# theogf/AugmentedGaussianProcesses.jl

Measured on AMD Instinct MI355X. Metric: cavi_iters_per_sec, higher is better.
Workload: dtype f64

## Files before the change

### augmentedgaussianprocesses.jl_amd/csrc/agp_chol.h

```cpp
#pragma once
#include "agp_cavi.h"
#include "agp_device.h"

namespace agp {

constexpr int LDP = TILE + 2;
constexpr int CHOL_THREADS = 512;

__device__ __forceinline__ double rcp1(double p) {
  double r = __builtin_amdgcn_rcp(p);
  return fma(r, fma(-p, r, 1.0), r);
}
__device__ __forceinline__ double rsqrt1(double p) {
  double y = __builtin_amdgcn_rsq(p);
  const double h = 0.5 * p;
  y = y * fma(-h * y, y, 1.5);
  y = y * fma(-h * y, y, 1.5);
  return y;
}
__device__ __forceinline__ float rsqrt1(float p) {
  float y = __builtin_amdgcn_rsqf(p);
  const float h = 0.5f * p;
  y = y * fmaf(-h * y, y, 1.5f);
  return y;
// ... 953 lines not shown

__global__ void k_wait_ge_fast(const int32_t* __restrict__ p, int32_t want, int32_t* __restrict__ info) {
  if (threadIdx.x != 0) return;
  long spins = 0;
  while ((int32_t)(__hip_atomic_load(p, __ATOMIC_RELAXED, __HIP_MEMORY_SCOPE_SYSTEM) - want) < 0) {
    __builtin_amdgcn_s_sleep(8);
    if (++spins > (1L << 27)) {
      atomicExch(info, -2);
      break;
    }
  }
}

__device__ __forceinline__ void dag_signal(int32_t* flag, int32_t epoch) {
  __builtin_amdgcn_fence(__ATOMIC_RELEASE, "workgroup");
  __syncthreads();
  if (threadIdx.x == 0) __hip_atomic_store(flag, epoch, __ATOMIC_RELAXED, __HIP_MEMORY_SCOPE_AGENT);
}

template <typename T>
__device__ __forceinline__ typename Mfma<T>::acc_t mma_tile16(const T* Ar, const T* Bc, int kend,
                                                              typename Mfma<T>::acc_t acc, bool neg, int lane) {
  const T* pa = Ar + (lane & 15) * LDP + (lane >> 4);
  const T* pb = Bc + (lane & 15) * LDP + (lane >> 4);
  typename Mfma<T>::acc_t p1;
#pragma unroll
  for (int r = 0; r < 4; ++r) p1[r] = T(0);
#pragma unroll 2
  for (int kk = 0; kk < kend / 4; kk += 2) {
    T a0 = pa[kk * 4], a1 = pa[kk * 4 + 4];
    const T b0 = pb[kk * 4], b1 = pb[kk * 4 + 4];
    if (neg) {
      a0 = -a0;
      a1 = -a1;
    }
    acc = Mfma<T>::mma(a0, b0, acc);
    p1 = Mfma<T>::mma(a1, b1, p1);
  }
#pragma unroll
  for (int r = 0; r < 4; ++r) acc[r] += p1[r];
  return acc;
}

template <typename T, typename F>
__device__ __forceinline__ void subst_tile(T* Ts, T* Xs, T* G, F after_first) {
  typedef typename Mfma<T>::acc_t acc_t;
  const int lane = threadIdx.x & 63, wave = threadIdx.x >> 6, ri = wave & 3, cj = wave >> 2;
  T* rowt = Ts + 16 * ri * LDP;
  T* own1 = rowt + 16 * cj;
  T* own2 = own1 + 32;
  const T* xlow = Xs + (32 + 16 * cj) * LDP;
  T* urow = Xs + 16 * (ri & 1) * LDP + 32 * (ri >> 1);
  auto emit = [&](int col0, acc_t v) {
    if (G) {
#pragma unroll
      for (int r = 0; r < 4; ++r)
        __hip_atomic_store(G + (16 * ri + Mfma<T>::row(lane, r)) * TILE + col0 + (lane & 15), v[r], __ATOMIC_RELAXED,
                           __HIP_MEMORY_SCOPE_AGENT);
    }
  };
  acc_t a;
#pragma unroll
  for (int r = 0; r < 4; ++r) a[r] = T(0);
  a = mma_tile16<T>(rowt, Xs + 16 * cj * LDP, 16 * (cj + 1), a, false, lane);
  after_first();
  acc_store16<T>(own1, a, lane);
  emit(16 * cj, a);
  __syncthreads();
  a = acc_load16<T>(own2, lane);
  a = mma_tile16<T>(rowt, xlow, 32, a, true, lane);
  acc_store16<T>(urow + 16 * cj, a, lane);
  __syncthreads();
#pragma unroll
  for (int r = 0; r < 4; ++r) a[r] = T(0);
  a = mma_tile16<T>(urow, xlow + 32, 16 * (cj + 1), a, false, lane);
  acc_store16<T>(own2, a, lane);
  emit(32 + 16 * cj, a);
}

template <typename T>
constexpr bool dag_feed_deferred() {
  return sizeof(T) == 8;
}
template <typename T, bool DEFER = dag_feed_deferred<T>()>
struct ChainPrefetch {
  const T* src;
  T *dT, *dD;
  int* bad;
  const int32_t *f1, *f2;
  int32_t epoch;
  int* ok;
  const T* dgsrc;
  T* gDg;
  const T* lsrc;
  T* gL;
  int ld_i;
  bool coh = false;
  int test = 0;
  T v[TILE * TILE / 256];
  __device__ __forceinline__ void operator()(int round) {
    int t = (int)threadIdx.x - 256;
    if (t < 0) return;
    if (sizeof(T) == 8) asm volatile("" : "+v"(t));
    if (round < 2) {
      if (dgsrc) {
#pragma unroll
        for (int q = 0; q < TILE * TILE / 512; ++q) {
          const int e = t + (2 * q + round) * 256;
          if (coh) __hip_atomic_store(gDg + e, dgsrc[(e >> 6) * LDP + (e & 63)], __ATOMIC_RELAXED, __HIP_MEMORY_SCOPE_AGENT);
          else gDg[e] = dgsrc[(e >> 6) * LDP + (e & 63)];
        }
      }
      return;
    }
    if (round < 4 && lsrc) {
#pragma unroll
      for (int q = 0; q < TILE * TILE / 512; ++q) {
        const int e = t + (2 * q + (round - 2)) * 256;
        gL[(e >> 6) * ld_i + (e & 63)] = lsrc[(e >> 6) * LDP + (e & 63)];
      }
    }
    if (!src) return;
    if (round == 3) {
      if (t == 0)
        *ok = (__hip_atomic_load(f1, __ATOMIC_RELAXED, __HIP_MEMORY_SCOPE_AGENT) == epoch) &&
              (__hip_atomic_load(f2, __ATOMIC_RELAXED, __HIP_MEMORY_SCOPE_AGENT) == epoch) && !(test & 2);
      return;
    }
    if (round < 4 || round > 6 || !*ok) return;
    if (round >= 5) {
      T* d = round == 5 ? dT : dD;
#pragma unroll
      for (int q = 0; q < TILE * TILE / 256; ++q) {
        const int e = t + q * 256;
        if (is_sent<T>(v[q])) *bad = 1;
        d[(e >> 6) * LDP + (e & 63)] = v[q];
      }
    }
    if (round <= 5) {
      const T* g = round == 4 ? src : src + TILE * TILE;
#pragma unroll
      for (int q = 0; q < TILE * TILE / 256; ++q)
        v[q] = __hip_atomic_load(g + t + q * 256, __ATOMIC_RELAXED, __HIP_MEMORY_SCOPE_AGENT);
    }
  }
  static __device__ __forceinline__ unsigned sent_away(T x) {
    typedef typename Sent<T>::U U;
    return (unsigned)(__builtin_bit_cast(U, x) >> (8 * sizeof(U) - 32)) ^ (unsigned)(Sent<T>::bits >> (8 * sizeof(U) - 32));
  }
  template <int HB>
  __device__ __forceinline__ void half(int rr) {
    if (!DEFER) {
      (*this)(HB + rr);
      return;
    }
    int t = (int)threadIdx.x - 256;
    if (t < 0) return;
    asm volatile("" : "+v"(t));
    if (HB == 0) {
      if (rr < 2) {
        if (dgsrc) {
#pragma unroll
          for (int q = 0; q < TILE * TILE / 512; ++q) {
            const int e = t + (2 * q + rr) * 256;
            if (coh) __hip_atomic_store(gDg + e, dgsrc[(e >> 6) * LDP + (e & 63)], __ATOMIC_RELAXED, __HIP_MEMORY_SCOPE_AGENT);
            else gDg[e] = dgsrc[(e >> 6) * LDP + (e & 63)];
          }
        }
        return;
      }
      if (lsrc) {
#pragma unroll
        for (int q = 0; q < TILE * TILE / 512; ++q) {
          const int e = t + (2 * q + (rr - 2)) * 256;
          gL[(e >> 6) * ld_i + (e & 63)] = lsrc[(e >> 6) * LDP + (e & 63)];
        }
      }
      if (src && rr == 3 && t == 0)
        *ok = (__hip_atomic_load(f1, __ATOMIC_RELAXED, __HIP_MEMORY_SCOPE_AGENT) == epoch) &&
              (__hip_atomic_load(f2, __ATOMIC_RELAXED, __HIP_MEMORY_SCOPE_AGENT) == epoch) && !(test & 2);
      return;
    }
    if (!src || (rr != 0 && rr != 3) || !*ok) return;
    if (rr == 3) {
      T* d = dT + (t >> 6) * LDP + (t & 63);
      unsigned away = ~0u;
#pragma unroll
      for (int q = 0; q < TILE * TILE / 256; ++q) {
        away = min(away, sent_away(v[q]));
        d[q * 4 * LDP] = v[q];
      }
      if (away == 0) *bad = 1;
    }
    const T* g = rr == 0 ? src : src + TILE * TILE;
#pragma unroll
    for (int q = 0; q < TILE * TILE / 256; ++q)
      v[q] = __hip_atomic_load(g + t + q * 256, __ATOMIC_RELAXED, __HIP_MEMORY_SCOPE_AGENT);
  }
  __device__ __forceinline__ void store_d() {
    int t = (int)threadIdx.x - 256;
    if (t < 0) return;
    asm volatile("" : "+v"(t));
    const T* g = src + TILE * TILE + t;
    const bool again = (test & 1) != 0;
    unsigned away = ~0u;
#pragma unroll
    for (int q = 0; q < TILE * TILE / 256; ++q) away = min(away, sent_away(v[q]));
    T* d = dD + (t >> 6) * LDP + (t & 63);
    if (away == 0 || again) {
#pragma unroll
      for (int q = 0; q < TILE * TILE / 256; ++q)
        d[q * 4 * LDP] = hv_settle<T>(g + q * 256, again ? __builtin_bit_cast(T, Sent<T>::bits) : v[q]);
    } else {
#pragma unroll
      for (int q = 0; q < TILE * TILE / 256; ++q) d[q * 4 * LDP] = v[q];
    }
  }
};

typedef unsigned int u32x4 __attribute__((ext_vector_type(4)));
__device__ __forceinline__ u32x4 load16_sc1(const void* p) {
  u32x4 v;
  asm volatile("global_load_dwordx4 %0, %1, off sc1" : "=v"(v) : "v"(p) : "memory");
  return v;
}
__device__ __forceinline__ void wait_vmcnt0() { asm volatile("s_waitcnt vmcnt(0)" ::: "memory"); }
template <typename T>
__device__ __forceinline__ T vec16_elem(u32x4 v, int i);
template <>
__device__ __forceinline__ double vec16_elem<double>(u32x4 v, int i) {
  const unsigned long long u = ((unsigned long long)v[2 * i + 1] << 32) | v[2 * i];
  return __builtin_bit_cast(double, u);
}
template <>
__device__ __forceinline__ float vec16_elem<float>(u32x4 v, int i) {
  return __builtin_bit_cast(float, (unsigned int)v[i]);
}
template <typename T>
__device__ __forceinline__ int pro_slot_off(int tid, int e) {
  constexpr int VEC = 16 / (int)sizeof(T);
  return (e / VEC) * (CHOL_THREADS * VEC) + tid * VEC + (e % VEC);
}

template <typename T>
struct EpiArgs {
  int on = 0;
  int64_t B = 0;
  int nslices = 0;
  const T* pk = nullptr;
  int64_t ldp = 0;
  T kdiag = T(0);
  const T* kd_ptr = nullptr;
  int use_kt = 0;
  T jitter = T(0), rho = T(0);
  LikParams<T> lp{};
  const T* y = nullptr;
  const int64_t* idx = nullptr;
  T *Kt = nullptr, *muf = nullptr, *varf = nullptr, *cb = nullptr, *theta = nullptr, *r = nullptr, *w = nullptr;
  int* flags = nullptr;
  const T* lam = nullptr;
  T* gamma = nullptr;
};

// ... 61 lines not shown
    }
#pragma unroll
    for (int r = 0; r < 4; ++r) red[wave * 256 + Mfma<T>::row(lane, r) * 16 + (lane & 15)] = acc[r];
    __syncthreads();
    if (threadIdx.x < 256) {
      const int e = threadIdx.x;
      T v = red[e];
#pragma unroll
      for (int o = 1; o < NW; ++o) v += red[o * 256 + e];
      out[(int64_t)(sl * PRO_PRE_KS + q) * TILE * TILE + (16 * bi + (e >> 4)) * TILE + 16 * bj + (e & 15)] = v;
    }
    __syncthreads();
  }
}

constexpr int ARRIVE_STRIDE = 16;
__device__ __forceinline__ void pro_arrival_gate(const int32_t* arrive, int g, int32_t want, int32_t* info) {
  if (threadIdx.x == 0) {
    long spins = 0;
    while ((int32_t)(__hip_atomic_load(arrive + g * ARRIVE_STRIDE, __ATOMIC_RELAXED, __HIP_MEMORY_SCOPE_AGENT) - want) < 0) {
      __builtin_amdgcn_s_sleep(8);
      if (++spins > (1L << 23)) {
        atomicExch(info, -4);
        break;
      }
    }
  }
  __syncthreads();
  __builtin_amdgcn_fence(__ATOMIC_ACQUIRE, "agent");
}

constexpr int PRO_NEAR = 4;
__host__ __device__ __forceinline__ int64_t pro_nhelp(int64_t nt, int64_t c, int ks, int kf) {
  const int64_t ntc = nt - c, nn = ntc < PRO_NEAR ? ntc : PRO_NEAR;
  return nn * (kf - 1) + (ntc - nn) * (ks - 1);
}
template <typename T>
__device__ __forceinline__ void pro_slice(const T* __restrict__ kap, int64_t ldk, const T* __restrict__ w, int64_t R0, int64_t c0,
                                          int64_t q0, int64_t q1, T* sm, Acc8<T>& acc) {
  constexpr int Q = TILE * TILE / CHOL_THREADS;
  const int r = threadIdx.x & 63, kb = threadIdx.x >> 6;
  const bool dg = R0 == c0;
  T va[Q], vb[Q], wv[Q];
  auto ldg = [&](int64_t qc) {
    const T* __restrict__ p = kap + (qc * TILE) * ldk;
#pragma unroll
    for (int q = 0; q < Q; ++q) {
      const int k = kb + 8 * q;
      va[q] = p[k * ldk + R0 + r];
      vb[q] = dg ? T(0) : p[k * ldk + c0 + r];
      wv[q] = w[qc * TILE + k];
    }
  };
  if (q0 < q1) ldg(q0);
  int cur = 0;
  for (int64_t qc = q0; qc < q1; ++qc) {
    T* As = sm + cur * 2 * TILE * LDP;
    T* Bs = As + TILE * LDP;
#pragma unroll
    for (int q = 0; q < Q; ++q) {
      const int k = kb + 8 * q;
      As[r * LDP + k] = va[q] * wv[q];
      Bs[r * LDP + k] = dg ? va[q] : vb[q];
    }
    __syncthreads();
    if (qc + 1 < q1) ldg(qc + 1);
    mma8<T>(As, Bs, acc);
    cur ^= 1;
  }
  __syncthreads();
}

constexpr long long CHAIN_GO_TICKS = 4LL * 100000000LL;
#ifndef AGP_TILES_WAVES_F64
#define AGP_TILES_WAVES_F64 4
#endif
#ifndef AGP_TILES_WAVES_F32
#define AGP_TILES_WAVES_F32 6
#endif
template <typename T, bool STEP, bool BATCH>
constexpr bool dag_block_subst() {
  return STEP && !BATCH && sizeof(T) == 8;
}
template <typename T, int ROLE, bool PRO>
constexpr int dag_min_waves() {
  return ROLE != 2 ? 1 : PRO ? (sizeof(T) == 8 ? 2 : 4) : (sizeof(T) == 8 ? AGP_TILES_WAVES_F64 : AGP_TILES_WAVES_F32);
}
template <typename T>
struct ProdArgs {
  T* out = nullptr;
  int64_t ld = 0;
  int64_t base = 0;
  T* fill = nullptr;
  int64_t fill_n = 0;
  double* ld_out = nullptr;
  int32_t* status = nullptr;
};

constexpr int STRACE_SLOTS = 8192, STRACE_XPUB = 600, STRACE_EXT = 1100, STRACE_FILL0 = 1400, STRACE_FILL1 = 1500, STRACE_WG0 = 2048,
              STRACE_WG1 = 4096, STRACE_MAXWG = 2048, STRACE_SAFE0 = 6144, STRACE_SAFE1 = 6400;
#ifdef AGP_STEP_TRACE
struct StraceExit {
  unsigned long long* p;
  __device__ ~StraceExit() {
    if (p && threadIdx.x == 0) *p = wall_clock64();
  }
};
#define STRACE(i) \
  if (PRO && ROLE == 0 && trace && threadIdx.x == 0) trace[i] = wall_clock64()
#else
#define STRACE(i)
#endif

template <typename T, bool FUSED, bool BATCH = false, bool TRACE = false, bool STEP = false, bool PRO = false, int ROLE = 0>
__global__ __launch_bounds__(CHOL_THREADS, (dag_min_waves<T, ROLE, PRO>()))
void k_chol_dag(CholBatch<T> bt, int nb, int64_t fstride, int64_t ld, int64_t ldx,
                                                           int64_t lde, int64_t ne, int64_t nt,
                                                           int32_t* __restrict__ info, int64_t nvalid, int32_t* flags,
                                                           int32_t epoch, unsigned long long* trace, T* H, int64_t hstride,
                                                           int64_t nx_, const T* __restrict__ erow, int opts, DagSync sync,
                                                           ProArgs<T> pro = ProArgs<T>{}, EpiArgs<T> epi = EpiArgs<T>{},
                                                           ProdArgs<T> prod = ProdArgs<T>{}) {
  static_assert(!PRO || (FUSED && !BATCH), "the prologue exists for single-problem launches with a chain workgroup only");
  static_assert(ROLE == 0 || (FUSED && STEP && !TRACE), "the split launch exists for the CAVI step's launches");
  const int64_t nx = STEP ? 0 : nx_;
  constexpr bool SUBST = dag_block_subst<T, STEP, BATCH>();
  const int write_x = STEP ? 0 : (opts & 1);
  const bool store_l = STEP ? false : (opts & 2) != 0;
  const int prob = BATCH ? (int)(blockIdx.x % (unsigned)nb) : 0;
  const int64_t bidx = BATCH ? (int64_t)(blockIdx.x / (unsigned)nb) : (int64_t)blockIdx.x;
  T* A = bt.A[prob];
  T* X = bt.X[prob];
  T* __restrict__ Dg = bt.Dg[prob];
  T* E = bt.E[prob];
  if (BATCH) erow = bt.R[prob];
  flags += prob * fstride;
  constexpr int64_t SLOT = TILE * TILE;
  T* HX = H + prob * hstride;
  T* HP = HX + nt * SLOT;
  T* HL = HP + 2 * nt * SLOT;
  __shared__ __attribute__((aligned(16))) T sm[((FUSED && ROLE != 2) || PRO ? 4 : 2) * TILE * LDP];
  __shared__ __attribute__((aligned(16))) T sc[(ROLE == 2 && !PRO) ? TILE : SC_ELEMS];
  __shared__ T piv[TILE];
  __shared__ int wait_ok, pf_ok, pf_bad;
  if (ROLE == 1) {
    if (threadIdx.x == 0) {
      wait_ok = 1;
      if (sync.here) __hip_atomic_fetch_add(sync.here, 1, __ATOMIC_RELAXED, __HIP_MEMORY_SCOPE_SYSTEM);
      unsigned spins = 0;
      const long long t0 = (long long)wall_clock64();
      while (sync.go) {
        const int32_t d = (int32_t)(__hip_atomic_load(sync.go, __ATOMIC_RELAXED, __HIP_MEMORY_SCOPE_SYSTEM) - sync.go_val);
        if (d == 0) break;
        if (d > 0) {
          wait_ok = 0;
          break;
        }
        __builtin_amdgcn_s_sleep(4);
        if ((++spins & 1023u) == 0 && (long long)wall_clock64() - t0 > CHAIN_GO_TICKS) {
          atomicExch(info, -1);
          wait_ok = 0;
#ifdef AGP_DEBUG_PTRS
          atomicAdd(&agp_dag_diag[5], 1ull);
#endif
          break;
        }
      }
    }
    __syncthreads();
    if (!wait_ok) {
      chain_count_out(sync);
      return;
    }
    __builtin_amdgcn_fence(__ATOMIC_ACQUIRE, "agent");
  }
  T* bufA = sm;
  T* bufB = sm + TILE * LDP;
  const int tid = threadIdx.x;
#ifdef AGP_STEP_TRACE
  StraceExit strace_exit{(PRO && ROLE == 0 && trace && bidx < STRACE_MAXWG) ? trace + STRACE_WG1 + bidx : nullptr};
  if (bidx < STRACE_MAXWG) STRACE(STRACE_WG0 + bidx);
#endif
  int64_t b = bidx, c = 0;
  bool helper = false;
  int64_t hbase = 0;
  const bool is_prod = !BATCH && !STEP && ROLE != 1 && prod.out != nullptr && bidx >= prod.base;
  static_assert(ROLE == 0 || STEP, "product workgroups (ProdArgs) must reach their sentinel refill unconditionally: ROLE 0 only");
  if (is_prod) {
    b = 0;
  } else if (PRO && ROLE == 1) {
  } else if (PRO) {
    for (;;) {
      if (c == nt) {
        const T sv = __builtin_bit_cast(T, Sent<T>::bits);
        if (b < 64) STRACE(STRACE_FILL0 + b);
        for (int64_t i = b * CHOL_THREADS + tid; i < pro.fill_n; i += (int64_t)pro.nfill * CHOL_THREADS) pro.fill[i] = sv;
        if (b < 64) STRACE(STRACE_FILL1 + b);
        return;
      }
      const int64_t nh = pro_nhelp(nt, c, pro.ks[c], pro.kf[c]), ntile = nt - c + ne + (nx ? c + 1 : 0);
      if (b < nh) {
        helper = true;
        break;
      }
      b -= nh;
      if (b < ntile) break;
      b -= ntile;
      hbase += nh;
      ++c;
// ... 36 lines not shown
  T* rowp = idr ? nullptr : ext ? E + (R - nt) * TILE * lde : A + R * TILE * ld;
  const int64_t ldr = ext ? lde : ld, c0 = c * TILE;
  int32_t* ready = flags;
  int32_t* xready = flags + (nt + ne + nx) * nt * DAG_FS;
  int32_t* pre1 = xready + nt * DAG_FS;
  int32_t* pre2 = pre1 + nt * DAG_FS;
  int32_t* abortf = pre2 + nt * DAG_FS;
#define DAG_TR(slot) \
  if (TRACE && tid == 0) trace[bidx * 8 + (slot)] = wall_clock64()
#define DAG_TRC(col, slot) \
  if (TRACE && tid == 0) trace[chain_slot(col, nt, ne, nx) * 8 + (slot)] = wall_clock64()
  if (is_prod) {
    const int64_t pidx = bidx - prod.base, nprod = nt * (nt + 1) / 2;
    if (prod.fill) {
      const T sv = __builtin_bit_cast(T, Sent<T>::bits);
      for (int64_t i = pidx * CHOL_THREADS + tid; i < prod.fill_n; i += nprod * CHOL_THREADS) prod.fill[i] = sv;
    }
    int64_t pi, pj;
    tri_index(pidx, pi, pj);
    const bool pdiag = pi == pj;
    const int64_t Ri = nt + ne + pi, Rj = nt + ne + pj;
    Acc8<T> pacc;
    pacc.zero();
    for (int64_t k = pi; k < nt; ++k) {
      if (!dag_wait(ready + (Ri * nt + k) * DAG_FS, pdiag ? nullptr : ready + (Rj * nt + k) * DAG_FS, epoch, abortf, info, &wait_ok))
        return;
      if (pdiag) load_tile_lds_hv<T>(HL + (Ri * nt + k) * SLOT, bufA);
      else load_tiles_lds_hv2<T>(HL + (Ri * nt + k) * SLOT, bufA, HL + (Rj * nt + k) * SLOT, bufB);
      __syncthreads();
      mma8<T>(bufA, pdiag ? bufA : bufB, pacc);
      __syncthreads();
    }
    const int64_t i0 = pi * TILE, j0 = pj * TILE;
    if (pdiag) {
      acc8_foreach<T>(pacc, [&](int r, int cc, T& val) { bufA[r * LDP + cc] = val; });
      __syncthreads();
      acc8_foreach<T>(pacc, [&](int r, int cc, T& val) {
        prod.out[(i0 + r) * prod.ld + i0 + cc] = cc > r ? bufA[cc * LDP + r] : val;
      });
    } else {
      acc8_foreach<T>(pacc, [&](int r, int cc, T& val) {
        prod.out[(i0 + r) * prod.ld + j0 + cc] = val;
        prod.out[(j0 + cc) * prod.ld + i0 + r] = val;
      });
    }
    if (prod.ld_out && pidx == nprod - 1) {
      __syncthreads();
      double lsum = 0.0;
      for (int64_t i = tid; i < nvalid; i += CHOL_THREADS) {
        const T* px = HX + (i / TILE) * SLOT + (i % TILE) * (TILE + 1);
        const T xv = hv_settle<T>(px, __hip_atomic_load(px, __ATOMIC_RELAXED, __HIP_MEMORY_SCOPE_AGENT));
        lsum -= log((double)xv);
      }
      lsum = block_sum<double>(lsum, reinterpret_cast<double*>(sc));
      if (tid == 0) {
        prod.ld_out[0] = lsum;
        int32_t* st_ = prod.status;
        if (st_) {
          const int32_t i0_ = __hip_atomic_load(st_, __ATOMIC_RELAXED, __HIP_MEMORY_SCOPE_AGENT);
          const int32_t i1_ = __hip_atomic_load(st_ + 1, __ATOMIC_RELAXED, __HIP_MEMORY_SCOPE_AGENT);
          const int32_t i2_ = __hip_atomic_load(st_ + 2, __ATOMIC_RELAXED, __HIP_MEMORY_SCOPE_AGENT);
          if (i1_ != 0 && st_[3] == 0) st_[3] = (i0_ != 0 || i2_ != 0) ? 2 : 1;
        }
      }
    }
    return;
  }
  DAG_TR(0);
  const bool chain = FUSED && c == 0 && b == 0;
  if (STEP && !BATCH && sync.started && chain && tid == 0 && ROLE != 1)
    __hip_atomic_store(sync.started, sync.seq, __ATOMIC_RELAXED, __HIP_MEMORY_SCOPE_SYSTEM);
  if (ROLE == 2 && chain) {
    if (tid == 0 && sync.go) __hip_atomic_store(sync.go, sync.go_val, __ATOMIC_RELAXED, __HIP_MEMORY_SCOPE_SYSTEM);
    if (!PRO) return;
  }
  if (ROLE == 1 && !chain) return;
  Acc8<T> acc;
  if (PRO && ROLE == 1) {
  } else if (PRO && !ext) {
    const int64_t ntc_ = nt - c, nn_ = ntc_ < PRO_NEAR ? ntc_ : PRO_NEAR;
    const bool pre = pro_pre_on<T>() && pro.pre && pro_pre_tile(R, c);
    const int ksc = pre ? 1 : b < nn_ ? pro.kf[c] : pro.ks[c];
    const int64_t nq = pro.Kdim / TILE;
    const int tsb = chain ? 0 : (R < 4 && c < 4) ? 64 + 8 * (4 * (int)R + (int)c) : 2040;
    PRO_TS(tsb);
    acc.zero();
    if (pre && pro.pre[PRO_PRE_VALID] == T(1)) {
      const T* __restrict__ pp = pro.pre + (R + c) * PRO_PRE_KS * TILE * TILE;
      T pv[PRO_PRE_KS][8];
      int e = 0;
      acc8_foreach<T>(acc, [&](int r, int cc, T& val) {
        (void)val;
#pragma unroll
        for (int q = 0; q < PRO_PRE_KS; ++q) pv[q][e] = pp[q * TILE * TILE + r * TILE + cc];
        ++e;
      });
      e = 0;
      acc8_foreach<T>(acc, [&](int r, int cc, T& val) {
        (void)r;
        (void)cc;
        T v = pv[0][e];
#pragma unroll
        for (int q = 1; q < PRO_PRE_KS; ++q) v += pv[q][e];
        val = v;
        ++e;
      });
    } else {
      pro_slice<T>(pro.kap, pro.ldk, pro.w, R * TILE, c0, 0, nq / ksc, sm, acc);
    }
    if (pro.packed) {
      if (pro.arrive) pro_arrival_gate(pro.arrive, pro.grp[c], pro.arrive_want, info);
      const T* __restrict__ tp = pro.packed + pack_index(R, c, nt) * (TILE * TILE);
      acc8_foreach<T>(acc, [&](int r, int cc, T& val) { val = tp[r * TILE + cc]; });
    }
    PRO_TS(tsb + 1);
    Acc8<T> e2v, kiv;
    acc8_foreach<T>(e2v, [&](int r, int cc, T& val) { val = pro.eta2[(R * TILE + r) * pro.ldm + c0 + cc]; });
    acc8_foreach<T>(kiv, [&](int r, int cc, T& val) { val = pro.Kinv[(R * TILE + r) * pro.ldm + c0 + cc]; });
    if (ksc > 1) {
      const int64_t h0 = hbase + (b < nn_ ? b * (pro.kf[c] - 1) : nn_ * (pro.kf[c] - 1) + (b - nn_) * (pro.ks[c] - 1));
      if (tid < ksc - 1) {
        long spins = 0;
        while (__hip_atomic_load(pro.sflags + (h0 + tid) * DAG_FS, __ATOMIC_RELAXED, __HIP_MEMORY_SCOPE_AGENT) != epoch) {
          __builtin_amdgcn_s_sleep(1);
          if (++spins > (1L << 28)) {
            atomicExch(info, -3);
            break;
          }
        }
      }
      __syncthreads();
      PRO_TS(tsb + 2);
      constexpr int VEC = 16 / (int)sizeof(T), NV = 8 / VEC;
      u32x4 pv[7][NV];
#pragma unroll
      for (int q = 0; q < 7; ++q)
        if (q < ksc - 1) {
          const T* hs = pro.HS + (h0 + q) * (TILE * TILE);
#pragma unroll
          for (int j = 0; j < NV; ++j) pv[q][j] = load16_sc1(hs + pro_slot_off<T>(tid, j * VEC));
        }
      wait_vmcnt0();
#pragma unroll
      for (int q = 0; q < 7; ++q)
        if (q < ksc - 1) {
          const T* hs = pro.HS + (h0 + q) * (TILE * TILE);
          int e = 0;
          acc8_foreach<T>(acc, [&](int r, int cc, T& val) {
            (void)r;
            (void)cc;
            const T got = vec16_elem<T>(pv[q][e / VEC], e % VEC);
            val += hv_settle<T>(hs + pro_slot_off<T>(tid, e), got);
            ++e;
          });
        }
    }
    PRO_TS(tsb + 3);
    if (pro.Cout) {
      int e = 0;
      acc8_foreach<T>(acc, [&](int r, int cc, T& val) {
        const T cv = val + T(0.25) * kiv.a[e >> 2][e & 3];
        ++e;
        pro.Cout[(R * TILE + r) * pro.ldm + c0 + cc] = cv;
        if (!diag) pro.Cout[(c0 + cc) * pro.ldm + R * TILE + r] = cv;
      });
    }
    {
// ... 6 lines not shown
        const T g = -(val + T(0.5) * kiv.a[mi][rr]) - e2;
        e2 += lr * g;
        val = e2;
      });
    }
    if (diag) {
      acc8_foreach<T>(acc, [&](int r, int cc, T& val) { bufA[r * LDP + cc] = val; });
      __syncthreads();
      acc8_foreach<T>(acc, [&](int r, int cc, T& val) {
        if (cc > r) val = bufA[cc * LDP + r];
        pro.eta2[(c0 + r) * pro.ldm + c0 + cc] = val;
        val *= T(-2);
      });
      __syncthreads();
    } else {
      acc8_foreach<T>(acc, [&](int r, int cc, T& val) {
        pro.eta2[(R * TILE + r) * pro.ldm + c0 + cc] = val;
        pro.eta2[(c0 + cc) * pro.ldm + R * TILE + r] = val;
        val *= T(-2);
      });
    }
    PRO_TS(tsb + 4);
  } else if (idr) {
    const bool on_diag = (R - nt - ne) == c;
    acc8_foreach<T>(acc, [&](int r, int cc, T& val) { val = (on_diag && r == cc) ? T(1) : T(0); });
  } else if (PRO && ext && R == nt + ne - 1) {
    if (pro.tred && pro.arrive) pro_arrival_gate(pro.arrive, 0, pro.arrive_want, info);
    const int col = tid & 63, grp = tid >> 6;
    T s0 = T(0), s1 = T(0), s2 = T(0), s3 = T(0);
    int64_t k = grp;
    for (; k + 24 < pro.Kdim; k += 32) {
      const T a0 = pro.kap[k * pro.ldk + c0 + col], a1 = pro.kap[(k + 8) * pro.ldk + c0 + col];
      const T a2 = pro.kap[(k + 16) * pro.ldk + c0 + col], a3 = pro.kap[(k + 24) * pro.ldk + c0 + col];
      s0 += a0 * pro.r[k];
      s1 += a1 * pro.r[k + 8];
      s2 += a2 * pro.r[k + 16];
      s3 += a3 * pro.r[k + 24];
    }
    for (; k < pro.Kdim; k += 8) s0 += pro.kap[k * pro.ldk + c0 + col] * pro.r[k];
    sc[grp * TILE + col] = (s0 + s1) + (s2 + s3);
    __syncthreads();
    if (grp == 0) {
      T t = T(0);
#pragma unroll
      for (int q = 0; q < CHOL_THREADS / 64; ++q) t += sc[q * TILE + col];
      if (pro.tred) t = pro.tred[c0 + col];
      T e = pro.eta1[c0 + col];
      e += pro.lr * (t + (pro.kinv_mu0 ? pro.kinv_mu0[c0 + col] : T(0)) - e);
      pro.eta1[c0 + col] = e;
      sc[CHOL_THREADS + col] = e;
    }
    __syncthreads();
    acc8_foreach<T>(acc, [&](int r, int cc, T& val) { val = r == 0 ? sc[CHOL_THREADS + cc] : T(0); });
    __syncthreads();
  } else if (erow && ext && R == nt + ne - 1) {
    acc8_foreach<T>(acc, [&](int r, int cc, T& val) { val = r == 0 ? erow[c0 + cc] : T(0); });
  } else {
    acc8_foreach<T>(acc, [&](int r, int cc, T& val) { val = rowp[r * ldr + c0 + cc]; });
  }
  if (PRO && ROLE == 2 && chain) {
    T* park = HP + SLOT;
    acc8_foreach<T>(acc, [&](int r, int cc, T& val) {
      __hip_atomic_store(park + r * TILE + cc, val, __ATOMIC_RELAXED, __HIP_MEMORY_SCOPE_AGENT);
    });
    dag_signal(pre2, epoch);
    return;
  }
  if (ROLE != 2 && chain) {
    if (PRO && ROLE == 1) {
      if (!dag_wait(pre2, nullptr, epoch, abortf, info, &wait_ok)) {
        chain_count_out(sync);
        return;
      }
      load_tile_lds_hv<T>(HP + SLOT, bufA);
    } else {
      acc8_foreach<T>(acc, [&](int r, int cc, T& val) { bufA[r * LDP + cc] = val; });
    }
    __syncthreads();
    T* bufC = sm + (FUSED ? 2 : 0) * TILE * LDP;
    T* bufD = sm + (FUSED ? 3 : 0) * TILE * LDP;
    for (int64_t k = 0; k < nt; ++k) {
      const int64_t k0 = k * TILE;
      T* trow = A + (k + 1) * TILE * ld;
      ChainPrefetch<T> pf;
      pf.src = k + 1 < nt ? HP + 2 * (k + 1) * SLOT : nullptr;
      pf.bad = &pf_bad;
      pf.dT = bufC;
      pf.dD = bufD;
      pf.f1 = pre1 + (k + 1) * DAG_FS;
      pf.f2 = pre2 + (k + 1) * DAG_FS;
      pf.epoch = epoch;
      pf.ok = &pf_ok;
      pf.dgsrc = k >= 1 ? bufD : nullptr;
      pf.gDg = Dg + (k - 1) * TILE * TILE;
      pf.lsrc = (k >= 1 && store_l) ? bufC : nullptr;
      pf.gL = A + k0 * ld + (k0 - TILE);
      pf.ld_i = (int)ld;
      pf.coh = ROLE == 1;
      pf.test = (opts >> 2) & 3;
      if (tid == 0) pf_ok = pf_bad = 0;
#ifdef AGP_STEP_TRACE
      PRO_TS(528 + k);
#endif
      factor_diag_tile_2lvl<T, ChainPrefetch<T>, SUBST>(bufA, bufB, sc, piv, info, k0, nvalid, pf);
      DAG_TRC(k, 2);
      PRO_TS(512 + k);
      {
        T xv[TILE * TILE / CHOL_THREADS];
        int tl = tid;
        asm volatile("" : "+v"(tl));
#pragma unroll
        for (int q = 0; q < TILE * TILE / CHOL_THREADS; ++q) {
          const int e = tl + q * CHOL_THREADS;
          xv[q] = bufB[(e >> 6) * LDP + (e & 63)];
        }
#pragma unroll
        for (int q = 0; q < TILE * TILE / CHOL_THREADS; ++q) {
          const int e = tl + q * CHOL_THREADS;
          __hip_atomic_store(HX + k * SLOT + e, xv[q], __ATOMIC_RELAXED, __HIP_MEMORY_SCOPE_AGENT);
          if (write_x) X[(k0 + (e >> 6)) * ldx + k0 + (e & 63)] = xv[q];
        }
      }
      if (k + 1 == nt) {
        for (int e = tid; e < TILE * TILE; e += CHOL_THREADS) {
          if (ROLE == 1) __hip_atomic_store(Dg + k * TILE * TILE + e, bufA[(e >> 6) * LDP + (e & 63)], __ATOMIC_RELAXED, __HIP_MEMORY_SCOPE_AGENT);
          else Dg[k * TILE * TILE + e] = bufA[(e >> 6) * LDP + (e & 63)];
        }
        dag_signal(xready + k * DAG_FS, epoch);
        DAG_TRC(k, 3);
        STRACE(STRACE_XPUB);
        if (ROLE == 1) chain_count_out(sync);
        return;
      }
      const bool late_feed = !pf_ok || pf_bad;
#ifdef AGP_STEP_TRACE
      if (PRO && trace && tid == 0) trace[560 + k] = !pf_ok ? 2ull : pf_bad ? 3ull : 1ull;
#endif
      if (late_feed) {
        dag_signal(xready + k * DAG_FS, epoch);
        DAG_TRC(k, 3);
        if (!dag_wait(pf.f1, pf.f2, epoch, abortf, info, &wait_ok)) {
          if (ROLE == 1) chain_count_out(sync);
          return;
        }
        load_tiles_lds_hv2<T>(HP + 2 * (k + 1) * SLOT, bufC, HP + (2 * (k + 1) + 1) * SLOT, bufD);
        __syncthreads();
      }
      if (TRACE && tid == 0) trace[chain_slot(k + 1, nt, ne, nx) * 8 + 7] = (unsigned long long)pf_ok;
      DAG_TRC(k + 1, 4);
      typedef typename Mfma<T>::acc_t acc_t;
      const int lane = tid & 63, wave = tid >> 6;
      if (SUBST) {
        subst_tile<T>(bufC, bufB, HL + ((k + 1) * nt + k) * SLOT, [&] {
          if (!late_feed) {
            dag_signal(xready + k * DAG_FS, epoch);
            DAG_TRC(k, 3);
          } else {
            __syncthreads();
          }
        });
      } else {
        const int ri = wave >> 1, cA = (wave & 1) ? 2 : 3, cB = 3 - cA;
        acc_t oa, ob;
#pragma unroll
        for (int r = 0; r < 4; ++r) oa[r] = ob[r] = T(0);
        oa = mma_tile16<T>(bufC + 16 * ri * LDP, bufB + 16 * cA * LDP, 16 * (cA + 1), oa, false, lane);
        ob = mma_tile16<T>(bufC + 16 * ri * LDP, bufB + 16 * cB * LDP, 16 * (cB + 1), ob, false, lane);
        if (!late_feed) {
          dag_signal(xready + k * DAG_FS, epoch);
          DAG_TRC(k, 3);
        } else {
          __syncthreads();
        }
#pragma unroll
        for (int r = 0; r < 4; ++r) {
          const int row = 16 * ri + Mfma<T>::row(lane, r);
          bufC[row * LDP + 16 * cA + (lane & 15)] = oa[r];
          bufC[row * LDP + 16 * cB + (lane & 15)] = ob[r];
          T* hl = HL + ((k + 1) * nt + k) * SLOT + row * TILE + (lane & 15);
          __hip_atomic_store(hl + 16 * cA, oa[r], __ATOMIC_RELAXED, __HIP_MEMORY_SCOPE_AGENT);
          __hip_atomic_store(hl + 16 * cB, ob[r], __ATOMIC_RELAXED, __HIP_MEMORY_SCOPE_AGENT);
        }
      }
      if (dag_feed_deferred<T>() && !late_feed) pf.store_d();
      __syncthreads();
      DAG_TRC(k + 1, 5);
      {
        const int ti_[10] = {0, 1, 1, 2, 2, 2, 3, 3, 3, 3}, tj_[10] = {0, 0, 1, 0, 1, 2, 0, 1, 2, 3};
#pragma unroll
        for (int rep = 0; rep < 2; ++rep) {
          const int tl = rep == 0 ? 2 + wave : wave;
          if (rep == 1 && wave >= 2) break;
          int i2 = 0, j2 = 0;
#pragma unroll
          for (int q = 0; q < 10; ++q)
            if (q == tl) {
              i2 = ti_[q];
              j2 = tj_[q];
            }
          acc_t a;
#pragma unroll
          for (int r = 0; r < 4; ++r) a[r] = bufD[(16 * i2 + Mfma<T>::row(lane, r)) * LDP + 16 * j2 + (lane & 15)];
          a = mma_tile16<T>(bufC + 16 * i2 * LDP, bufC + 16 * j2 * LDP, TILE, a, true, lane);
#pragma unroll
          for (int r = 0; r < 4; ++r) bufD[(16 * i2 + Mfma<T>::row(lane, r)) * LDP + 16 * j2 + (lane & 15)] = a[r];
        }
      }
      dag_signal(ready + ((k + 1) * nt + k) * DAG_FS, epoch);
      {
        T* t0 = bufA;
        bufA = bufD;
        bufD = t0;
      }
      DAG_TRC(k + 1, 1);
    }
    if (ROLE == 1) chain_count_out(sync);
    return;
  }
  if (ROLE == 1) return;
  const bool f1 = FUSED && b == 1 && !ext;
  const bool f2 = FUSED && diag;
  const int64_t jend = f2 ? c - 1 : c;
  const bool epi_row = PRO && epi.on && ext && !idr && c == nt - 1 && R < nt + ne - 1;
  T epi_ss = T(0), epi_dt = T(0), epi_sk = T(0), epi_y = T(0);
  const int er = tid >> 3, es = (tid & 7) * 8;
  if (epi_row) {
    const int64_t i = (R - nt) * TILE + er;
    if (!epi.use_kt && i < epi.B)
      for (int q = (tid & 7); q < epi.nslices; q += 8) epi_sk += epi.pk[q * epi.ldp + i];
    if ((tid & 7) == 0 && i < epi.B) epi_y = epi.y[epi.idx ? epi.idx[i] : i];
  }
  auto epi_acc = [&](const T* Wt , const T* vslot ) {
    if (tid < TILE) piv[tid] = hv_settle<T>(vslot + tid, __hip_atomic_load(vslot + tid, __ATOMIC_RELAXED, __HIP_MEMORY_SCOPE_AGENT));
    __syncthreads();
#pragma unroll
    for (int q = 0; q < 8; ++q) {
      const T a = Wt[er * LDP + es + q];
      epi_ss += a * a;
      epi_dt += a * piv[es + q];
    }
  };
  for (int64_t j = idr ? R - nt - ne : 0; j < jend; ++j) {
    if (!dag_wait(ready + (R * nt + j) * DAG_FS, diag ? nullptr : ready + (c * nt + j) * DAG_FS, epoch, abortf, info, &wait_ok))
      return;
    if (j == c - 1) DAG_TR(4);
    if (diag) load_tile_lds_hv<T>(HL + (R * nt + j) * SLOT, bufA);
    else load_tiles_lds_hv2<T>(HL + (R * nt + j) * SLOT, bufA, HL + (c * nt + j) * SLOT, bufB);
    __syncthreads();
    if (j == c - 1) DAG_TR(5);
    if (epi_row) epi_acc(bufA, HL + ((nt + ne - 1) * nt + j) * SLOT);
    mma8_sub<T>(bufA, diag ? bufA : bufB, acc);
    __syncthreads();
  }
  if (!f2) DAG_TR(1);
  if (f1 || f2) {
    T* park = f1 ? HP + 2 * (c + 1) * SLOT : HP + (2 * c + 1) * SLOT;
    acc8_foreach<T>(acc, [&](int r, int cc, T& val) {
      __hip_atomic_store(park + r * TILE + cc, val, __ATOMIC_RELAXED, __HIP_MEMORY_SCOPE_AGENT);
    });
    dag_signal((f1 ? pre1 + (c + 1) * DAG_FS : pre2 + c * DAG_FS), epoch);
    if (R < 4 && c < 4) PRO_TS(64 + 8 * (4 * (int)R + (int)c) + 5);
    if (f2) {
      DAG_TR(6);
    } else {
      DAG_TR(3);
    }
    return;
  }
  acc8_foreach<T>(acc, [&](int r, int cc, T& val) { bufA[r * LDP + cc] = val; });
  if (!FUSED && diag) {
    __syncthreads();
    factor_diag_tile_2lvl<T>(bufA, bufB, sc, piv, info, c0, nvalid);
    DAG_TR(2);
    for (int e = tid; e < TILE * TILE; e += CHOL_THREADS) {
      const int r = e >> 6, cc = e & 63;
      __hip_atomic_store(HX + c * SLOT + e, bufB[r * LDP + cc], __ATOMIC_RELAXED, __HIP_MEMORY_SCOPE_AGENT);
      X[(c0 + r) * ldx + c0 + cc] = bufB[r * LDP + cc];
    }
    dag_signal(xready + c * DAG_FS, epoch);
    for (int e = tid; e < TILE * TILE; e += CHOL_THREADS) Dg[c * TILE * TILE + e] = bufA[(e >> 6) * LDP + (e & 63)];
    DAG_TR(3);
    return;
  }
  if (!dag_wait(xready + c * DAG_FS, nullptr, epoch, abortf, info, &wait_ok)) return;
  DAG_TR(2);
  const bool strace_row = ext && !idr && c == nt - 1 && R - nt < 64;
  (void)strace_row;
  if (strace_row) STRACE(STRACE_EXT + 4 * (R - nt));
  load_tile_lds_hv<T>(HX + c * SLOT, bufB);
  __syncthreads();
  DAG_TR(6);
  Acc8<T> out;
  if (SUBST) {
    subst_tile<T>(bufA, bufB, (T*)nullptr, [] { __syncthreads(); });
    __syncthreads();
    acc8_foreach<T>(out, [&](int r, int cc, T& val) { val = bufA[r * LDP + cc]; });
  } else {
    out.zero();
    mma8<T>(bufA, bufB, out);
  }
  {
    T* hs = HL + (R * nt + c) * SLOT;
    acc8_foreach<T>(out, [&](int r, int cc, T& val) {
      __hip_atomic_store(hs + r * TILE + cc, val, __ATOMIC_RELAXED, __HIP_MEMORY_SCOPE_AGENT);
    });
  }
  if (idr) {
    const int64_t i0 = (R - nt - ne) * TILE;
    acc8_foreach<T>(out, [&](int r, int cc, T& val) { X[(c0 + cc) * ldx + i0 + r] = val; });
  } else if (ext || store_l) {
    acc8_foreach<T>(out, [&](int r, int cc, T& val) { rowp[r * ldr + c0 + cc] = val; });
  }
  DAG_TR(7);
  dag_signal(ready + (R * nt + c) * DAG_FS, epoch);
  DAG_TR(3);
  if (strace_row) STRACE(STRACE_EXT + 4 * (R - nt) + 1);
  if (epi_row) {
    if (!SUBST) {
      __syncthreads();
      acc8_foreach<T>(out, [&](int r, int cc, T& val) { bufA[r * LDP + cc] = val; });
      __syncthreads();
    }
    epi_acc(bufA, HL + ((nt + ne - 1) * nt + c) * SLOT);
    STRACE(STRACE_EXT + 4 * (R - nt) + 2);
    const int64_t i = (R - nt) * TILE + er;
    T sk = epi_sk;
#pragma unroll
    for (int o = 1; o < 8; o <<= 1) {
      epi_ss += __shfl_xor(epi_ss, o);
      epi_dt += __shfl_xor(epi_dt, o);
      sk += __shfl_xor(sk, o);
    }
    if ((tid & 7) == 0 && i < epi.B) {
      const T kd = epi.kdiag < T(0) ? epi.kd_ptr[0] : epi.kdiag;
      rowstats_finish<T>(i, epi_ss, epi_dt, sk, kd, epi.use_kt, epi.jitter, epi.rho, epi.lp, epi.y, epi.idx, epi.Kt, epi.muf,
                         epi.varf, epi.cb, epi.theta, epi.r, epi.w, epi.flags, epi.lam, epi.gamma, &epi_y);
    }
#ifdef AGP_STEP_TRACE
    __syncthreads();
    STRACE(STRACE_EXT + 4 * (R - nt) + 3);
#endif
  }
#undef DAG_TR
#undef DAG_TRC
// ... 64 lines not shown
```

### augmentedgaussianprocesses.jl_amd/csrc/agp_chol_host.h

```cpp
#pragma once
#include <cmath>
#include "agp_ctx.h"
#include "agp_linalg.h"

static agp_status tri_scratch_ensure(agp_ctx* c, size_t need) {
  if (c->tri_bytes < need) {
    if (c->tri_scratch) {
      (void)hipStreamSynchronize(c->stream);
      (void)hipFree(c->tri_scratch);
    }
    c->tri_scratch = nullptr;
    c->tri_bytes = 0;
    if (hipMalloc(&c->tri_scratch, need) != hipSuccess) return AGP_ERR_NOMEM;
    c->tri_bytes = need;
  }
  return AGP_OK;
}

template <typename T>
static agp_status trtri_levels(agp_ctx* c, const T* A, int64_t ld, T* X, int64_t ldx, int64_t nt) {
  if (nt <= 1) return AGP_OK;
  const int64_t n = nt * TILE;
  AGPCHK(tri_scratch_ensure(c, sizeof(T) * (size_t)n * (size_t)n));
  T* S = (T*)c->tri_scratch;
// ... 256 lines not shown
      } else {
        trail(c->stream, k0, k1, kn, nt);
      }
    }
  }
  if (side_busy) HIPCHK(c, hipStreamWaitEvent(c->stream, c->ev_join, 0));
  return AGP_OK;
}

static void dag_pause(agp_ctx* c) {
  c->dag_off = true;
  c->dag_cooldown = c->dag_backoff;
  c->dag_backoff = std::min<int64_t>(c->dag_backoff * 4, (int64_t)1 << 20);
}
static void dag_tick(agp_ctx* c) {
  if (c->dag_off && --c->dag_cooldown <= 0) c->dag_off = false;
}
static void dag_retry_check(agp_ctx* c) {
  if (!c->safe_retries || c->dag_off) return;
  int32_t r = 0;
  if (hipMemcpy(&r, c->safe_retries, sizeof(r), hipMemcpyDeviceToHost) != hipSuccess) return;
  if (r > c->dag_retries_seen) {
    fprintf(stderr,
            "[agp_hip] warning: %d task-graph factorisation(s) lost a tile dependency (is another process using this GPU?) and were "
            "re-run by the in-stream fallback; this context uses plain launches for the next %lld steps\n",
            (int)(r - c->dag_retries_seen), (long long)c->dag_backoff);
    c->dag_retries_seen = r;
    dag_pause(c);
  }
}

static bool chain_split_wanted(int64_t tiles, bool with_prologue = false, bool f64 = true) {
  static const int v = []() {
    const char* e = getenv("AGP_CHAIN_SPLIT");
    return e ? (e[0] == '0' ? 0 : 1) : -1;
  }();
  if (with_prologue && f64 && v < 0) return false;
  return v < 0 ? tiles >= 600 : v == 1;
}
static bool chain_split_ready(agp_ctx* c) {
  if (c->chain_state != 0) return c->chain_state == 1;
  c->chain_state = -1;
  int lo = 0, hi = 0;
  if (hipDeviceGetStreamPriorityRange(&lo, &hi) != hipSuccess) return false;
  if (hipStreamCreateWithPriority(&c->chain_stream, hipStreamNonBlocking, hi) != hipSuccess) {
    c->chain_stream = nullptr;
    (void)hipGetLastError();
    return false;
  }
  bool ok = hipExtMallocWithFlags((void**)&c->chain_go, 8, hipMallocSignalMemory) == hipSuccess && hipMemset(c->chain_go, 0, 8) == hipSuccess &&
            hipMalloc((void**)&c->chain_ctr, sizeof(int32_t)) == hipSuccess && hipMemset(c->chain_ctr, 0, sizeof(int32_t)) == hipSuccess;
  int32_t* hs = nullptr;
  ok = ok && hipMalloc((void**)&hs, 4 * sizeof(int32_t)) == hipSuccess && hipMemset(hs, 0, 4 * sizeof(int32_t)) == hipSuccess;
  if (ok) {
    (void)hipStreamSynchronize(c->stream);
    hipLaunchKernelGGL(k_handshake, dim3(1), dim3(64), 0, c->chain_stream, hs, (const int32_t*)(hs + 1), hs + 2);
    hipLaunchKernelGGL(k_handshake, dim3(1), dim3(64), 0, c->stream, hs + 1, (const int32_t*)hs, hs + 3);
    int32_t res[4] = {0, 0, 0, 0};
    ok = hipStreamSynchronize(c->chain_stream) == hipSuccess && hipStreamSynchronize(c->stream) == hipSuccess &&
         hipMemcpy(res, hs, sizeof(res), hipMemcpyDeviceToHost) == hipSuccess && res[2] == 1 && res[3] == 1;
  }
  if (hs) (void)hipFree(hs);
  (void)hipGetLastError();
  if (ok) c->chain_state = 1;
  return ok;
}
static void chain_split_arm(agp_ctx* c, DagSync& ds, int nb) {
  ds.go = c->chain_go;
  ds.go_val = ++c->chain_seq;
  ds.done = c->chain_ctr;
  ds.here = c->chain_go + 1;
  c->chain_exits += nb;
}
static void chain_split_wait_here(agp_ctx* c) {
  hipLaunchKernelGGL(k_wait_here, dim3(1), dim3(64), 0, c->stream, (const int32_t*)(c->chain_go + 1), c->chain_exits);
}

struct StepSync {
  DagSync ds{};
  bool used = false;
};

static void pro_ks_table(int64_t nt, int64_t nq, bool f64, unsigned char* ks, unsigned char* kf, bool pre = false) {
  const double tc = f64 ? 2.7 : 1.6, tau = f64 ? 17.8 : 14.0, head = pre ? 24.0 : 12.0;
  for (int64_t c = 0; c < nt && c < 32; ++c) {
    int want;
    if (c == 0) want = 8;
    else if (c == 1) want = f64 ? 4 : 8;
    else want = (int)std::ceil((double)nq * (tc + 0.3) / std::max(tau * (double)c - head, 1.0));
    want = std::max(1, std::min<int>(want, (int)std::min<int64_t>(8, nq)));
    ks[c] = kf[c] = (unsigned char)want;
  }
}
static bool dag_test_abort() {
  static const bool on = []() {
    const char* e = getenv("AGP_DAG_TEST_ABORT");
    return e && e[0] == '1';
  }();
  return on;
}

static int dag_test_feed() {
  static const int v = []() {
    const char* e = getenv("AGP_DAG_TEST_FEED");
    return e && e[0] == '1' ? 1 : e && e[0] == '2' ? 2 : 0;
  }();
  return v;
}

static agp_status dag_flags_ensure(agp_ctx* c, int64_t nf) {
  if (c->dag_cap < nf) {
    if (c->dag_flags) (void)hipFree(c->dag_flags);
    c->dag_flags = nullptr;
    c->dag_cap = 0;
    if (hipMalloc((void**)&c->dag_flags, sizeof(int32_t) * (size_t)(nf + 1024)) != hipSuccess) return AGP_ERR_NOMEM;
    c->dag_cap = nf + 1024;
    HIPCHK(c, hipMemsetAsync(c->dag_flags, 0, sizeof(int32_t) * (size_t)c->dag_cap, c->stream));
    c->dag_epoch = 0;
  }
  return AGP_OK;
}
template <typename T>
static bool dag_take_refill(agp_ctx* c, int other, T** fill, int64_t* fill_n) {
  auto& d = c->h_dirty[other];
  if (!(c->hset[other] && d.on && d.nb == 1 && c->htype == (int)sizeof(T))) return false;
  *fill = (T*)c->hset[other];
  *fill_n = d.used;
  d.on = false;
  return true;
}

template <bool BATCH_, bool STEP_, bool PRO_>
struct DagKernel { static constexpr bool BATCH = BATCH_, STEP = STEP_, PRO = PRO_; };
using DagFactor = DagKernel<false, false, false>;
using DagFactorPro = DagKernel<false, false, true>;
using DagStep = DagKernel<false, true, false>;
using DagStepPro = DagKernel<false, true, true>;
using DagStepBatch = DagKernel<true, true, false>;

template <typename T>
struct DagArgs {
  CholBatch<T> bt{};
  int nb = 1;
  int64_t fstride = 0, ld = 0, ldx = 0, lde = 0, ne = 0, nt = 0;
  int32_t* info = nullptr;
  int64_t nvalid = 0;
  unsigned long long* trace = nullptr;
  T* H = nullptr;
  int64_t hstride = 0, nx = 0;
  const T* erow = nullptr;
  int opts = 0;
  DagSync ds{};
  ProArgs<T> pro{};
  EpiArgs<T> epi{};
  ProdArgs<T> prod{};
};
template <typename T, typename K, int ROLE>
static void dag_enqueue(agp_ctx* c, unsigned grid, hipStream_t stream, const DagArgs<T>& a) {
  hipLaunchKernelGGL((k_chol_dag<T, true, K::BATCH, false, K::STEP, K::PRO, ROLE>), dim3(grid), dim3(CHOL_THREADS), 0, stream, a.bt,
                     a.nb, a.fstride, a.ld, a.ldx, a.lde, a.ne, a.nt, a.info, a.nvalid, c->dag_flags, c->dag_epoch, a.trace, a.H,
                     a.hstride, a.nx, a.erow, a.opts | (dag_test_feed() << 2), a.ds, a.pro, a.epi, a.prod);
}
template <typename T, typename K>
static agp_status dag_launch(agp_ctx* c, unsigned grid, bool split, DagArgs<T>& a) {
  if constexpr (K::STEP) {
    if (split) {
      chain_split_arm(c, a.ds, a.nb);
      dag_enqueue<T, K, 1>(c, (unsigned)a.nb, c->chain_stream, a);
      chain_split_wait_here(c);
      dag_enqueue<T, K, 2>(c, grid, c->stream, a);
      LAUNCHCHK(c);
      return AGP_OK;
    }
  }
// ... 181 lines not shown
```

Baseline: 3570.

## Skip Dg tile stores in f64 CAVI step and retune prologue K-split table

In the f64 CAVI step path, the chain workgroup no longer writes factored diagonal tiles to the Dg buffer, either in the prefetch helper or after the last tile. This removes global stores from the latency-critical Cholesky chain. The host prologue K-split table gets a new timing model for f64 with more than three tiles, with separate split counts for near and far rows. It also adds trace-only timestamps. The risk is that any consumer of Dg in the step path now reads stale data.

Result: faster. 3719 (median of 6 runs) (+4.2%).

```diff
diff --git a/augmentedgaussianprocesses.jl_amd/csrc/agp_chol.h b/augmentedgaussianprocesses.jl_amd/csrc/agp_chol.h
--- a/augmentedgaussianprocesses.jl_amd/csrc/agp_chol.h
+++ b/augmentedgaussianprocesses.jl_amd/csrc/agp_chol.h
@@ -1059,7 +1059,7 @@
 constexpr bool dag_feed_deferred() {
   return sizeof(T) == 8;
 }
-template <typename T, bool DEFER = dag_feed_deferred<T>()>
+template <typename T, bool DEFER = dag_feed_deferred<T>(), bool DG = true>
 struct ChainPrefetch {
   const T* src;
   T *dT, *dD;
@@ -1074,13 +1074,16 @@
   int ld_i;
   bool coh = false;
   int test = 0;
+#ifdef AGP_STEP_TRACE
+  unsigned long long* tlook = nullptr;
+#endif
   T v[TILE * TILE / 256];
   __device__ __forceinline__ void operator()(int round) {
     int t = (int)threadIdx.x - 256;
     if (t < 0) return;
     if (sizeof(T) == 8) asm volatile("" : "+v"(t));
     if (round < 2) {
-      if (dgsrc) {
+      if (DG && dgsrc) {
 #pragma unroll
         for (int q = 0; q < TILE * TILE / 512; ++q) {
           const int e = t + (2 * q + round) * 256;
@@ -1136,7 +1139,7 @@
     asm volatile("" : "+v"(t));
     if (HB == 0) {
       if (rr < 2) {
-        if (dgsrc) {
+        if (DG && dgsrc) {
 #pragma unroll
           for (int q = 0; q < TILE * TILE / 512; ++q) {
             const int e = t + (2 * q + rr) * 256;
@@ -1153,9 +1156,13 @@
           gL[(e >> 6) * ld_i + (e & 63)] = lsrc[(e >> 6) * LDP + (e & 63)];
         }
       }
-      if (src && rr == 3 && t == 0)
+      if (src && rr == 3 && t == 0) {
         *ok = (__hip_atomic_load(f1, __ATOMIC_RELAXED, __HIP_MEMORY_SCOPE_AGENT) == epoch) &&
               (__hip_atomic_load(f2, __ATOMIC_RELAXED, __HIP_MEMORY_SCOPE_AGENT) == epoch) && !(test & 2);
+#ifdef AGP_STEP_TRACE
+        if (tlook) *tlook = wall_clock64();
+#endif
+      }
       return;
     }
     if (!src || (rr != 0 && rr != 3) || !*ok) return;
@@ -1383,6 +1390,10 @@
 constexpr bool dag_block_subst() {
   return STEP && !BATCH && sizeof(T) == 8;
 }
+template <typename T, bool STEP, bool BATCH>
+constexpr bool dag_store_dg() {
+  return !(STEP && sizeof(T) == 8);
+}
 template <typename T, int ROLE, bool PRO>
 constexpr int dag_min_waves() {
   return ROLE != 2 ? 1 : PRO ? (sizeof(T) == 8 ? 2 : 4) : (sizeof(T) == 8 ? AGP_TILES_WAVES_F64 : AGP_TILES_WAVES_F32);
@@ -1399,7 +1410,7 @@
 };
 
 constexpr int STRACE_SLOTS = 8192, STRACE_XPUB = 600, STRACE_EXT = 1100, STRACE_FILL0 = 1400, STRACE_FILL1 = 1500, STRACE_WG0 = 2048,
-              STRACE_WG1 = 4096, STRACE_MAXWG = 2048, STRACE_SAFE0 = 6144, STRACE_SAFE1 = 6400;
+              STRACE_WG1 = 4096, STRACE_MAXWG = 2048, STRACE_SAFE0 = 6144, STRACE_SAFE1 = 6400, STRACE_LOOK = 608, STRACE_NEAR = 640;
 #ifdef AGP_STEP_TRACE
 struct StraceExit {
   unsigned long long* p;
@@ -1426,6 +1437,7 @@
   static_assert(ROLE == 0 || (FUSED && STEP && !TRACE), "the split launch exists for the CAVI step's launches");
   const int64_t nx = STEP ? 0 : nx_;
   constexpr bool SUBST = dag_block_subst<T, STEP, BATCH>();
+  constexpr bool STORE_DG = dag_store_dg<T, STEP, BATCH>();
   const int write_x = STEP ? 0 : (opts & 1);
   const bool store_l = STEP ? false : (opts & 2) != 0;
   const int prob = BATCH ? (int)(blockIdx.x % (unsigned)nb) : 0;
@@ -1628,7 +1640,12 @@
     const bool pre = pro_pre_on<T>() && pro.pre && pro_pre_tile(R, c);
     const int ksc = pre ? 1 : b < nn_ ? pro.kf[c] : pro.ks[c];
     const int64_t nq = pro.Kdim / TILE;
+#ifdef AGP_STEP_TRACE
+    const bool ts_near = !(R < 4 && c < 4) && c >= 2 && c <= 6 && b < PRO_NEAR;
+    const int tsb = chain ? 0 : (R < 4 && c < 4) ? 64 + 8 * (4 * (int)R + (int)c) : ts_near ? STRACE_NEAR + 8 * (4 * ((int)c - 2) + (int)b) : 2040;
+#else
     const int tsb = chain ? 0 : (R < 4 && c < 4) ? 64 + 8 * (4 * (int)R + (int)c) : 2040;
+#endif
     PRO_TS(tsb);
     acc.zero();
     if (pre && pro.pre[PRO_PRE_VALID] == T(1)) {
@@ -1801,7 +1818,7 @@
     for (int64_t k = 0; k < nt; ++k) {
       const int64_t k0 = k * TILE;
       T* trow = A + (k + 1) * TILE * ld;
-      ChainPrefetch<T> pf;
+      ChainPrefetch<T, dag_feed_deferred<T>(), STORE_DG> pf;
       pf.src = k + 1 < nt ? HP + 2 * (k + 1) * SLOT : nullptr;
       pf.bad = &pf_bad;
       pf.dT = bufC;
@@ -1810,7 +1827,7 @@
       pf.f2 = pre2 + (k + 1) * DAG_FS;
       pf.epoch = epoch;
       pf.ok = &pf_ok;
-      pf.dgsrc = k >= 1 ? bufD : nullptr;
+      pf.dgsrc = (STORE_DG && k >= 1) ? bufD : nullptr;
       pf.gDg = Dg + (k - 1) * TILE * TILE;
       pf.lsrc = (k >= 1 && store_l) ? bufC : nullptr;
       pf.gL = A + k0 * ld + (k0 - TILE);
@@ -1820,8 +1837,9 @@
       if (tid == 0) pf_ok = pf_bad = 0;
 #ifdef AGP_STEP_TRACE
       PRO_TS(528 + k);
+      pf.tlook = (PRO && trace) ? trace + STRACE_LOOK + k : nullptr;
 #endif
-      factor_diag_tile_2lvl<T, ChainPrefetch<T>, SUBST>(bufA, bufB, sc, piv, info, k0, nvalid, pf);
+      factor_diag_tile_2lvl<T, decltype(pf), SUBST>(bufA, bufB, sc, piv, info, k0, nvalid, pf);
       DAG_TRC(k, 2);
       PRO_TS(512 + k);
       {
@@ -1841,9 +1859,11 @@
         }
       }
       if (k + 1 == nt) {
-        for (int e = tid; e < TILE * TILE; e += CHOL_THREADS) {
-          if (ROLE == 1) __hip_atomic_store(Dg + k * TILE * TILE + e, bufA[(e >> 6) * LDP + (e & 63)], __ATOMIC_RELAXED, __HIP_MEMORY_SCOPE_AGENT);
-          else Dg[k * TILE * TILE + e] = bufA[(e >> 6) * LDP + (e & 63)];
+        if (STORE_DG) {
+          for (int e = tid; e < TILE * TILE; e += CHOL_THREADS) {
+            if (ROLE == 1) __hip_atomic_store(Dg + k * TILE * TILE + e, bufA[(e >> 6) * LDP + (e & 63)], __ATOMIC_RELAXED, __HIP_MEMORY_SCOPE_AGENT);
+            else Dg[k * TILE * TILE + e] = bufA[(e >> 6) * LDP + (e & 63)];
+          }
         }
         dag_signal(xready + k * DAG_FS, epoch);
         DAG_TRC(k, 3);
@@ -1979,6 +1999,9 @@
     });
     dag_signal((f1 ? pre1 + (c + 1) * DAG_FS : pre2 + c * DAG_FS), epoch);
     if (R < 4 && c < 4) PRO_TS(64 + 8 * (4 * (int)R + (int)c) + 5);
+#ifdef AGP_STEP_TRACE
+    if (!(R < 4 && c < 4) && c >= 2 && c <= 6) PRO_TS(STRACE_NEAR + 8 * (4 * ((int)c - 2) + (int)b) + 5);
+#endif
     if (f2) {
       DAG_TR(6);
     } else {
diff --git a/augmentedgaussianprocesses.jl_amd/csrc/agp_chol_host.h b/augmentedgaussianprocesses.jl_amd/csrc/agp_chol_host.h
--- a/augmentedgaussianprocesses.jl_amd/csrc/agp_chol_host.h
+++ b/augmentedgaussianprocesses.jl_amd/csrc/agp_chol_host.h
@@ -362,14 +362,23 @@
 };
 
 static void pro_ks_table(int64_t nt, int64_t nq, bool f64, unsigned char* ks, unsigned char* kf, bool pre = false) {
-  const double tc = f64 ? 2.7 : 1.6, tau = f64 ? 17.8 : 14.0, head = pre ? 24.0 : 12.0;
-  for (int64_t c = 0; c < nt && c < 32; ++c) {
-    int want;
-    if (c == 0) want = 8;
-    else if (c == 1) want = f64 ? 4 : 8;
-    else want = (int)std::ceil((double)nq * (tc + 0.3) / std::max(tau * (double)c - head, 1.0));
-    want = std::max(1, std::min<int>(want, (int)std::min<int64_t>(8, nq)));
-    ks[c] = kf[c] = (unsigned char)want;
+  const int cap = (int)std::min<int64_t>(8, nq);
+  auto split = [&](double work, double budget) { return std::max(1, std::min(cap, (int)std::ceil(work / std::max(budget, 1.0)))); };
+  if (nt <= 3 || !f64) {
+    const double tc = f64 ? 2.7 : 1.6, tau = f64 ? 17.8 : 14.0, head = pre ? 24.0 : 12.0;
+    for (int64_t c = 0; c < nt && c < 32; ++c)
+      ks[c] = kf[c] = (unsigned char)(c == 0 ? cap : c == 1 ? std::min(cap, f64 ? 4 : 8) : split((double)nq * (tc + 0.3), tau * (double)c - head));
+    return;
+  }
+  const double tc = 3.4, tau = 16.2, tu = 4.0, te = 4.0, tl = 6.0, ts0 = 7.0, ts1 = 2.5, margin = 3.0, f0 = pre ? 17.4 : 27.4;
+  const double slope = tau - tu - ts1;
+  const double head_near = 2.0 * tau - 2.0 * tu + ts0 + te + margin - tl - f0;
+  const double head_far = head_near - (tau + tl - tu - margin);
+  kf[0] = (unsigned char)cap, ks[0] = (unsigned char)std::min(cap, 4);
+  kf[1] = ks[1] = (unsigned char)std::min(cap, 4);
+  for (int64_t c = 2; c < nt && c < 32; ++c) {
+    kf[c] = (unsigned char)split((double)nq * tc, slope * (double)c - head_near);
+    ks[c] = (unsigned char)split((double)nq * tc, slope * (double)c - head_far);
   }
 }
 static bool dag_test_abort() {
```
